# vislearn/esac

Measured on AMD Instinct MI355X. Metric: pose hypotheses/sec @640x480, 256 hyp, higher is better.
Workload: dtype f64 (P3P, LM refinement, exact decisions) + f32 (streaming soft-inlier score, ranking only); 1 GPU; BASELINE configs[1]: 1 expert(s), 256 hypotheses in total (256 per GPU), 60x80 grid (sub-sampling 8 of a 640x480 frame), all hypotheses on the one expert; tau=10 alpha=100 beta=0.5 maxReproj=100; box-room frames, 2 cm noise, 30% outliers; experts=1, hypotheses_total=256, frames_cycled=16, policy=range

## Files before the change

### esac_amd/api.py

```python
import ctypes as C
import os
import threading

import numpy as np
import torch

from . import build as _build

RES_SCORE, RES_HYP, RES_EXPERT, RES_RVEC, RES_TVEC, RES_POSE = 0, 1, 2, 3, 6, 9
RES_REF_STEPS, RES_INLIERS, RES_PROB, RES_ENTROPY, RES_CONTENDERS, RES_LM_ITERS, RES_DOUBLES = 25, 26, 27, 28, 29, 30, 32
BUF_HYPS, BUF_SAMPLE_XY, BUF_TRIES, BUF_SCORES, BUF_RESULT = 0, 1, 2, 3, 4
BUF_INLIER_MAP, BUF_INLIER_COUNTS, BUF_WINNER_ERRS, BUF_EXACT_FLAGS, BUF_CYCLES = 5, 6, 7, 8, 9
BUF_BWD_PROBS, BUF_BWD_LOSSES, BUF_BWD_REF_HYPS, BUF_BWD_SCORE_GRADS, BUF_BWD_SLOTS, BUF_BWD_SLOT_INFO, BUF_BWD_DLOSS = \
    10, 11, 12, 13, 14, 15, 16
BUF_BWD_PATH1, BUF_BWD_PATH2 = 17, 18
BUF_REFINE_INFO = 19
BUF_BWD_TEAM_INFO = 20
BUF_SPEC_INFO = 21
BUF_SPEC_FLAGS = 22
REFINE_TEAM_MAX, REFINE_TEAM_EIGHT, REFINE_TEAM_AUTO = 32, 8, -1
REFINE_TEAM_DEFAULT = REFINE_TEAM_AUTO
MAX_REF_STEPS = 100
BWD_MAX_SLOTS = 1000

ABI_SYMBOLS = [
    "esac_hip_abi_version", "esac_hip_last_error", "esac_hip_device_count", "esac_hip_create", "esac_hip_destroy",
    "esac_hip_forward", "esac_hip_sample", "esac_hip_score", "esac_hip_select", "esac_hip_refine",
    "esac_hip_score_exact", "esac_hip_read", "esac_hip_write_hyps", "esac_hip_phase_ms", "esac_hip_set_timing",
    "esac_hip_score_span_ms", "esac_hip_forward_batch", "esac_hip_backward", "esac_hip_set_debug", "esac_hip_check",
    "esac_hip_pick_record", "esac_hip_time_stages", "esac_hip_shard_balanced", "esac_hip_set_wait",
    "esac_hip_set_refine_team", "esac_hip_host_turn",
    "esac_hip_comm_unique_id", "esac_hip_comm_init", "esac_hip_comm_destroy", "esac_hip_allreduce_sum", "esac_hip_comm_info",
    "esac_hip_host_turn_mean", "esac_hip_backward_batch",
    "esac_hip_forward_batch_cams", "esac_hip_backward_batch_cams",
]
COMM_ID_BYTES = 128
ABI_VERSION = 6
FLAG_EXACT_SCORES, FLAG_SCORE_TILED, FLAG_SCORE_STREAM, FLAG_PACK_MAPS, FLAG_EXACT_SAMPLING, FLAG_SCORES_BY_INDEX = 1, 2, 4, 8, 16, 32
FLAG_AUTO_EXACT = 64
FLAG_REFINE_SOLO = 128
FLAG_STRICT_REFERENCE = 256
FLAG_STRICT_TRAINING = 512
WAIT_SPIN, WAIT_YIELD, WAIT_BLOCK = 0, 1, 2
DEBUG_ERROR_IMAGE, DEBUG_COOP_STALL, DEBUG_TEAM_SPREAD, DEBUG_NO_SPECULATION, DEBUG_SPEC_SECOND_BEST, DEBUG_SPEC_LOSE_CHAIN = 1, 2, 4, 8, 16, 32


class Params(C.Structure):
    _fields_ = [
        ("E", C.c_int32), ("H", C.c_int32), ("W", C.c_int32), ("N", C.c_int32),
        ("shift_x", C.c_int32), ("shift_y", C.c_int32),
        ("focal", C.c_float), ("ppx", C.c_float), ("ppy", C.c_float),
        ("inlier_thresh", C.c_float), ("inlier_alpha", C.c_float), ("inlier_beta", C.c_float),
        ("max_reproj", C.c_float), ("sub_sampling", C.c_int32),
        ("seed", C.c_uint64), ("call", C.c_uint64),
        ("max_tries", C.c_int32), ("max_ref_steps", C.c_int32), ("hyp_offset", C.c_int32),
        ("rescore_margin", C.c_float),
        ("d_hyp_index", C.c_void_p),
        ("flags", C.c_int32),
        ("expert_base", C.c_int32),
    ]


class FrameCam(C.Structure):
    _fields_ = [
        ("shift_x", C.c_int32), ("shift_y", C.c_int32),
        ("focal", C.c_float), ("ppx", C.c_float), ("ppy", C.c_float),
        ("reserved", C.c_int32 * 3),
    ]


CAM_DTYPE = np.dtype([("shift_x", np.int32), ("shift_y", np.int32), ("focal", np.float32), ("ppx", np.float32),
                      ("ppy", np.float32), ("reserved", np.int32, (3,))])


def make_cams(shift_x, shift_y, focal, ppx, ppy):
    B = len(shift_x)
    cams = np.zeros(B, CAM_DTYPE)
# ... 314 lines not shown

    def pick_record(self, records, world, zero=None):
        assert records.is_cuda and records.dtype == torch.float64 and records.is_contiguous() and records.numel() >= 32 * world
        assert zero is None or (zero.is_cuda and zero.dtype == torch.float64 and zero.is_contiguous())
        rc = self.lib.esac_hip_pick_record(self.ctx, records.data_ptr(), int(world), self._stream(), self._host_addr,
                                           zero.data_ptr() if zero is not None else None, int(zero.numel()) if zero is not None else 0)
        if rc != 0:
            _check(rc, self.lib)
        return self._host_np.copy()

    def shard_balanced(self, hyp_assign, world, rank, E, expert_base=0, index_out=None, assign_out=None, info_out=None):
        assert hyp_assign.is_cuda and hyp_assign.dtype == torch.int64 and hyp_assign.is_contiguous()
        N = int(hyp_assign.shape[0])
        n_local = N // world + (1 if rank < N % world else 0)
        dev = self.device
        if index_out is None:
            index_out = torch.empty(max(n_local, 1), dtype=torch.int32, device=dev)
        if assign_out is None:
            assign_out = torch.empty(max(n_local, 1), dtype=torch.int64, device=dev)
        if info_out is None:
            info_out = torch.empty(4, dtype=torch.int32, device=dev)
        self._call(self.lib.esac_hip_shard_balanced, hyp_assign.data_ptr(), N, int(E), int(world), int(rank), int(expert_base),
                   self._stream(), index_out.data_ptr(), assign_out.data_ptr(), info_out.data_ptr())
        self._keep_shard = (hyp_assign, index_out, assign_out, info_out)
        return index_out[:n_local], assign_out[:n_local], info_out

    def set_wait(self, mode):
        _check(self.lib.esac_hip_set_wait(self.ctx, int(mode)), self.lib)

    def check(self):
        _check(self.lib.esac_hip_check(self.ctx), self.lib)

    def set_debug(self, keep_error_image=False, coop_stall=False, team_spread=False, no_speculation=False, spec_second_best=False,
                  spec_lose_chain=False):
        _check(self.lib.esac_hip_set_debug(self.ctx, (DEBUG_ERROR_IMAGE if keep_error_image else 0) | (DEBUG_COOP_STALL if coop_stall else 0) |
                                           (DEBUG_TEAM_SPREAD if team_spread else 0) | (DEBUG_NO_SPECULATION if no_speculation else 0) |
                                           (DEBUG_SPEC_SECOND_BEST if spec_second_best else 0) | (DEBUG_SPEC_LOSE_CHAIN if spec_lose_chain else 0)), self.lib)

    def spec_info(self):
        v = self.read(BUF_SPEC_INFO)
        return {"calls": int(v[0]), "failures": int(v[1]), "last_speculative": bool(v[2]), "last_failed": bool(v[3])}

    def set_refine_team(self, members=REFINE_TEAM_DEFAULT):
        _check(self.lib.esac_hip_set_refine_team(self.ctx, int(members)), self.lib)

    def bwd_team_info(self):
        v = self.read(BUF_BWD_TEAM_INFO)
        return {"teams": bool(v[0]), "team_calls": int(v[1]), "team_fallbacks": int(v[2]), "slots": int(v[3])}

    def refine_info(self):
        v = self.read(BUF_REFINE_INFO)
        return {"mode": ("one_workgroup", "cooperating", "team")[int(v[0])] if 0 <= int(v[0]) <= 2 else int(v[0]),
                "workgroups": int(v[1]),
                "xcd_census": [(int(v[2]) >> (8 * x)) & 255 for x in range(4)] + [(int(v[7]) >> (8 * x)) & 255 for x in range(4)],
                "same_xcd": bool(v[3]),
                "exchanges": int(v[4]), "timed_out": bool(v[5]), "team_fallbacks": int(v[6]) & 0x3fffffff,
                "team_latched_off": bool(int(v[6]) & 0x40000000)}

    def comm_unique_id(self):
        buf = (C.c_ubyte * COMM_ID_BYTES)()
        _check(self.lib.esac_hip_comm_unique_id(buf, COMM_ID_BYTES), self.lib)
        return bytes(buf)

    def comm_init(self, nranks, rank, unique_id):
        assert len(unique_id) == COMM_ID_BYTES
        buf = (C.c_ubyte * COMM_ID_BYTES).from_buffer_copy(unique_id)
        _check(self.lib.esac_hip_comm_init(self.ctx, int(nranks), int(rank), buf, COMM_ID_BYTES), self.lib)
        self._comm = (int(nranks), int(rank))

    def comm_destroy(self):
# ... 308 lines not shown
```

### esac_amd/csrc/esac_capi.hip

```cpp
#include <hip/hip_runtime.h>
#include <dlfcn.h>
#include <sched.h>
#include <time.h>
#include <stdarg.h>
#include <stddef.h>
#include <stdio.h>
#include <stdlib.h>
#include <string.h>

#include "../../include/esac_hip.h"
#include "esac_kernels.hpp"
#include "pose_math.hpp"

using namespace esac;

extern "C" {
typedef struct ncclComm* ncclComm_t;
typedef struct { char internal[128]; } ncclUniqueId;
typedef int ncclResult_t;
}

static_assert(ESAC_RES_SCORE == ESAC_RES_SCORE_K && ESAC_RES_HYP == ESAC_RES_HYP_K && ESAC_RES_EXPERT == ESAC_RES_EXPERT_K &&
                  ESAC_RES_RVEC == ESAC_RES_RVEC_K && ESAC_RES_POSE == ESAC_RES_POSE_K &&
                  ESAC_RES_REF_STEPS == ESAC_RES_REF_STEPS_K && ESAC_RES_INLIERS == ESAC_RES_INLIERS_K &&
// ... 71 lines not shown
    int last_nsel = 0;
    bool slot_teams = true;
    long long slot_team_calls = 0, slot_team_fallbacks = 0;
    bool last_bwd_teams = false;
    BwdArgs bws{};
    int bP = 0, bcap = 0;
    long long bN = 0, bslots = 0, brows = 0;
    int bB = 0;
    bool b_lists = false;
    int bcap_batch = 0;
    long long bwd_budget = 2048LL << 20;
    int last_bwd_frames = 1;
    int last_bwd_batch_cap = 0;
    double* h_gt = nullptr;
    double* d_gt = nullptr;
    FrameCam* h_cams = nullptr;
    FrameCam* d_cams = nullptr;
    hipEvent_t cams_ev = nullptr;
    bool cams_queued = false;
    float4* sc4 = nullptr;
    long long sc4_cells = 0;
    int tN = 0, tChunks = 0;
    long long tPart = 0;
    bool rt32_stale = false;
    double host_ns[8] = {0, 0, 0, 0, 0, 0, 0, 0};
    double host_sum[8] = {0, 0, 0, 0, 0, 0, 0, 0};
    double host_last_return = 0;
    long long host_n = 0;
    hipStream_t side = nullptr;
    hipStream_t side2 = nullptr;
    bool spec_off = false, spec_env_off = false;
    bool spec_second_best = false;
    bool spec_lose_chain = false;
    long long spec_calls = 0;
    double last_spec_epoch = 0;
    ncclComm_t comm = nullptr;
    int comm_ranks = 0, comm_rank = 0;
};

static inline double now_ns() {
    timespec ts;
    clock_gettime(CLOCK_MONOTONIC, &ts);
    return (double)ts.tv_sec * 1e9 + (double)ts.tv_nsec;
}

extern "C" int esac_hip_abi_version(void) { return ESAC_HIP_ABI_VERSION; }
extern "C" const char* esac_hip_last_error(void) { return g_err; }
extern "C" int esac_hip_device_count(void) {
    int n = 0;
    if (hipGetDeviceCount(&n) != hipSuccess) return 0;
    return n;
}

constexpr int ESAC_SLOT_TEAMS_MAX = 32;
constexpr int ESAC_TEAM_STRIKES = 2;
constexpr long long ESAC_TEAM_REARM_CALLS = 1000;

static_assert(sizeof(ncclUniqueId) == ESAC_COMM_ID_BYTES, "unique id size");
constexpr ncclResult_t ncclSuccess = 0;
constexpr int NCCL_SUM = 0, NCCL_DOUBLE = 8;
struct Rccl {
    ncclResult_t (*get_unique_id)(ncclUniqueId*) = nullptr;
    ncclResult_t (*comm_init_rank)(ncclComm_t*, int, ncclUniqueId, int) = nullptr;
    ncclResult_t (*comm_destroy)(ncclComm_t) = nullptr;
    ncclResult_t (*all_reduce)(const void*, void*, size_t, int, int, ncclComm_t, hipStream_t) = nullptr;
    const char* (*error_string)(ncclResult_t) = nullptr;
// ... 554 lines not shown
        KArgs as = a;
        as.spec_mode = 1;
        as.result_user = nullptr;
        as.result_pin = nullptr;
        launch_score(as, s);
        if ((rc = check_launch("k_score_fast (settled)"))) return rc;
        c->host_ns[2] = now_ns() - t_entry;
        if (tm) HIP_OK(hipEventRecord(c->ev[2], s));
        if (tm) HIP_OK(hipEventRecord(c->ev[3], s));
        KArgs ar = as;
        ar.spec_mode = 2;
        ar.spec_debug = c->spec_second_best ? 1 : 0;
        c->refine_tag = launch_refine(ar, s);
        c->refine_was_team = refine_team_members(ar) > 0;
        if ((rc = check_launch("k_refine (speculative)"))) return rc;
        launch_spec_wait(a, 3, c->side2);
        launch_select_rescore(as, c->side2);
        if ((rc = check_launch("k_select_rescore (settled)"))) return rc;
        launch_spec_wait(a, 3, c->side);
        launch_sample_stragglers_on(chain, chain_waves, c->side);
        if (!c->spec_lose_chain) launch_score_stragglers(a, c->side);
        if ((rc = check_launch("straggler chain"))) return rc;
        launch_spec_join(a, c->side2);
        if ((rc = check_launch("k_spec_join"))) return rc;
        {
            KArgs ag = a;
            ag.spec_gate = 1;
            const unsigned long long tag2 = launch_refine(ag, s);
            (void)tag2;
            if ((rc = check_launch("k_refine (gated)"))) return rc;
        }
        c->host_ns[3] = now_ns() - t_entry;
    } else {
        launch_sample(a, s);
        if ((rc = check_launch("k_sample"))) return rc;
        c->host_ns[1] = now_ns() - t_entry;
        if (tm) HIP_OK(hipEventRecord(c->ev[1], s));
        if (exact) launch_rescore_all(a, s);
        else       launch_score(a, s);
        if ((rc = check_launch(exact ? "k_rescore(all)" : "k_score_fast"))) return rc;
        c->host_ns[2] = now_ns() - t_entry;
        if (tm) HIP_OK(hipEventRecord(c->ev[2], s));
        a.fold_select = !c->fold_select ? 0 : refine_folds_select(a) ? 1 : refine_folds_exact_stats(a) ? 2 : 0;
        if (exact) {
            if (a.fold_select != 2) launch_stats_exact(a, s);
        } else if (!a.fold_select) {
            launch_select_rescore(a, s);
        }
        if ((rc = check_launch(exact ? "k_stats_exact" : "k_select_rescore"))) return rc;
        if (tm) HIP_OK(hipEventRecord(c->ev[3], s));
        c->refine_tag = launch_refine(a, s);
        c->refine_was_team = refine_team_members(a) > 0;
        if ((rc = check_launch("k_refine"))) return rc;
        c->host_ns[3] = now_ns() - t_entry;
    }
    if (tm) {
        HIP_OK(hipEventRecord(c->ev[4], s));
        HIP_OK(hipEventRecord(c->ev[5], s));
        HIP_OK(hipEventRecord(c->ev[6], s));
        c->ev_valid = true;
    }
    if (h_result_out) {
        if ((rc = wait_record(c, s, B, c->epoch, "esac_hip_forward: the refinement kernel"))) return rc;
        if (spec_ok && c->h_pin[33] == 5.0) {
            c->spec_off = c->spec_env_off = true;
            HIP_OK(hipStreamSynchronize(c->side));
            if (c->side2) HIP_OK(hipStreamSynchronize(c->side2));
            HIP_OK(hipStreamSynchronize(s));
            return forward_impl(c, d_sc, sc_frame_stride, d_assign, p, B, stream, d_scores_out, d_result_out, h_result_out);
        }
        c->host_ns[4] = now_ns() - t_entry;
        bool team_failed = false;
// ... 49 lines not shown
    for (int k = 0; k < 6; k++) out_ns[k] = c->host_sum[k] / n;
    out_ns[6] = c->host_n > 1 ? c->host_sum[6] / (double)(c->host_n - 1) : 0.0;
    out_ns[7] = (double)c->host_n;
    if (reset) {
        for (double& v : c->host_sum) v = 0;
        c->host_n = 0;
        c->host_last_return = 0;
    }
    return 0;
}

extern "C" int esac_hip_host_turn(esac_hip_ctx* c, double out_ns[8]) {
    if (!c || !out_ns) return fail(-1, "esac_hip_host_turn: null argument");
    for (int k = 0; k < 8; k++) out_ns[k] = c->host_ns[k];
    return 0;
}

extern "C" int esac_hip_time_stages(esac_hip_ctx* c, const float* d_sc, const int64_t* d_assign, const esac_hip_params* p,
                                    void* stream, int reps, float out_ms[4]) {
    if (!c || !out_ms || reps < 1) return fail(-1, "esac_hip_time_stages: bad argument");
    DeviceGuard guard(c->device);
    KArgs a;
    int rc = make_args(c, d_sc, d_assign, p, &a);
    if (rc) return rc;
    a.tstamps = nullptr;
    forward_team(c, a);
    hipStream_t s = (hipStream_t)stream;
    c->rt32_stale = false;
    mark_sampling(c, a);
    if ((a.flags & ESAC_FLAG_AUTO_EXACT) && a.E == 1 && (long long)a.N * a.H * a.W <= ESAC_AUTO_EXACT_MAX_WORK)
        a.flags |= ESAC_FLAG_EXACT_SCORES | ESAC_FLAG_EXACT_SAMPLING;
    const bool exact = (a.flags & ESAC_FLAG_EXACT_SCORES) != 0;
    a.fold_select = !c->fold_select ? 0 : refine_folds_select(a) ? 1 : refine_folds_exact_stats(a) ? 2 : 0;
    auto stage = [&](int k) {
        switch (k) {
            case 0: launch_sample(a, s); break;
            case 1: if (exact) launch_rescore_all(a, s); else launch_score(a, s); break;
            case 2: if (exact) { if (a.fold_select != 2) launch_stats_exact(a, s); } else if (!a.fold_select) launch_select_rescore(a, s); break;
            default: c->refine_tag = launch_refine(a, s); break;
        }
    };
    for (int k = 0; k < 4; k++) stage(k);
    if ((rc = check_launch("forward chain"))) return rc;
    hipEvent_t ev[8];
    for (auto& e : ev) HIP_OK(hipEventCreate(&e));
    for (int k = 0; k < 4; k++) {
        stage(k);
        HIP_OK(hipEventRecord(ev[2 * k], s));
        for (int r = 0; r < reps; r++) stage(k);
        HIP_OK(hipEventRecord(ev[2 * k + 1], s));
    }
    if ((rc = check_launch("stage timing"))) return rc;
    HIP_OK(hipEventSynchronize(ev[7]));
    for (int k = 0; k < 4; k++) {
        HIP_OK(hipEventElapsedTime(&out_ms[k], ev[2 * k], ev[2 * k + 1]));
        out_ms[k] /= (float)reps;
    }
    for (auto& e : ev) (void)hipEventDestroy(e);
    return 0;
}

extern "C" int esac_hip_pick_record(esac_hip_ctx* c, const double* d_records, int world, void* stream, double* h_record_out, double* d_zero,
                                    int n_zero) {
    if (!c || !d_records || !h_record_out || world < 1 || n_zero < 0 || (n_zero > 0 && !d_zero))
        return fail(-1, "esac_hip_pick_record: bad argument");
    DeviceGuard guard(c->device);
    hipStream_t s = (hipStream_t)stream;
    c->epoch += 1.0;
    const double want = c->epoch;
// ... 562 lines not shown

extern "C" int esac_hip_write_hyps(esac_hip_ctx* c, const double* h_hyps, int N) {
    if (!c || !h_hyps || N <= 0) return fail(-1, "esac_hip_write_hyps: bad argument");
    DeviceGuard guard(c->device);
    int rc = ensure_ws(c, N, c->capP > 0 ? c->capP : 1);
    if (rc) return rc;
    HIP_OK(hipDeviceSynchronize());
    HIP_OK(hipMemcpy(c->ws.hyps, h_hyps, (size_t)N * 6 * sizeof(double), hipMemcpyHostToDevice));
    c->rt32_stale = true;
    c->lastN = N;
    return 0;
}

extern "C" int esac_hip_set_refine_team(esac_hip_ctx* c, int members) {
    if (!c) return fail(-1, "null context");
    if (members < ESAC_REFINE_TEAM_AUTO || members > ESAC_REFINE_TEAM_MAX)
        return fail(-4, "esac_hip_set_refine_team: %d members (0..%d, or ESAC_REFINE_TEAM_AUTO)", members, ESAC_REFINE_TEAM_MAX);
    c->team_auto = members == ESAC_REFINE_TEAM_AUTO && !c->team_auto_env_off;
    c->team = members == ESAC_REFINE_TEAM_AUTO ? ESAC_REFINE_TEAM_DEFAULT : members < 2 ? 0 : members;
    c->team_latched_off = false;
    c->team_strikes = 0;
    c->slot_teams = true;
    return 0;
}

extern "C" int esac_hip_set_debug(esac_hip_ctx* c, int flags) {
    if (!c) return fail(-1, "null context");
    c->keep_errs = (flags & ESAC_DEBUG_ERROR_IMAGE) != 0;
    c->coop_stall = (flags & ESAC_DEBUG_COOP_STALL) != 0;
    c->team_spread = (flags & ESAC_DEBUG_TEAM_SPREAD) != 0;
    c->spec_off = c->spec_env_off || (flags & ESAC_DEBUG_NO_SPECULATION) != 0;
    c->spec_second_best = (flags & ESAC_DEBUG_SPEC_SECOND_BEST) != 0;
    c->spec_lose_chain = (flags & ESAC_DEBUG_SPEC_LOSE_CHAIN) != 0;
    return 0;
}

extern "C" int esac_hip_set_timing(esac_hip_ctx* c, int enabled) {
    if (!c) return fail(-1, "null context");
    c->timing = enabled != 0;
    c->timing_period = enabled > 1 ? enabled : 1;
    c->timing_calls = 0;
    c->ev_valid = false;
    if (c->ws.span_acc) {
        DeviceGuard guard(c->device);
        HIP_OK(hipDeviceSynchronize());
        HIP_OK(hipMemset(c->ws.span_acc, 0, 2 * sizeof(long long)));
    }
    return 0;
}

extern "C" int esac_hip_phase_ms(esac_hip_ctx* c, float out[6]) {
    if (!c || !out) return fail(-1, "esac_hip_phase_ms: null argument");
    if (!c->timing || !c->ev_valid) return fail(-8, "esac_hip_phase_ms: timing is off or no forward has run");
    DeviceGuard guard(c->device);
    HIP_OK(hipEventSynchronize(c->ev[4]));
    for (int i = 0; i < 4; i++) HIP_OK(hipEventElapsedTime(&out[i], c->ev[i], c->ev[i + 1]));
    HIP_OK(hipEventElapsedTime(&out[4], c->ev[0], c->ev[4]));
    HIP_OK(hipEventSynchronize(c->ev[6]));
    HIP_OK(hipEventElapsedTime(&out[5], c->ev[5], c->ev[6]));
    return 0;
}

extern "C" int esac_hip_score_span_ms(esac_hip_ctx* c, float* mean_ms, int* launches) {
    if (!c || !mean_ms) return fail(-1, "esac_hip_score_span_ms: null argument");
    if (!c->ws.span_acc) return fail(-8, "esac_hip_score_span_ms: no forward has run");
    DeviceGuard guard(c->device);
// ... 8 lines not shown
```

### esac_amd/csrc/esac_kernels.hip

```cpp
#include <hip/hip_runtime.h>
#include <stdint.h>
#include <stdlib.h>

#include "pose_math.hpp"
#include "p3p_screen.hpp"
#include "rng.hpp"
#include "esac_kernels.hpp"
#include "device_common.hpp"

namespace esac {

__device__ __forceinline__ bool accept_sample(const double Rp[9], const double Tp[3], const float (&Pf)[4][3], const double (&mu)[4],
                                              const double (&mv)[4], const Cam& cam, double tau, double rvec[3], double T[3],
                                              double R[9]) {
    rodrigues_mat2vec(Rp, rvec);
    rodrigues_vec2mat<false>(rvec, R, nullptr);
    T[0] = Tp[0]; T[1] = Tp[1]; T[2] = Tp[2];
    bool accepted = true;
#pragma unroll
    for (int j = 0; j < 4; j++) {
        const double Xd = Pf[j][0], Yd = Pf[j][1], Zd = Pf[j][2];
        double x = R[0] * Xd + R[1] * Yd + R[2] * Zd + T[0];
        double y = R[3] * Xd + R[4] * Yd + R[5] * Zd + T[1];
        double z = R[6] * Xd + R[7] * Yd + R[8] * Zd + T[2];
// ... 1014 lines not shown
        double R[9];
#pragma unroll
        for (int k = 0; k < 9; k++) R[k] = a.hyps_R[(size_t)h * 9 + k];
        double acc[1] = {0};
        for (int i = threadIdx.x; i < P; i += B) {
            const int row = i / a.W, col = i - row * a.W;
            float err = project_exact_err(R, t, cam, mx[i], mx[P + i], mx[2 * P + i], cell_px(a, col), cell_py(a, row));
            if (STRICT) err = a.max_reproj < err ? a.max_reproj : err;
            else        err = err < a.max_reproj ? err : a.max_reproj;
            acc[0] += soft_inlier_exact(err, a.tau, a.beta);
        }
        block_sum<1, B>(acc, s_part, s_tot);
        if (threadIdx.x == 0) {
            const float scale = a.alpha / a.W / a.H;
            double s = acc[0];
            s *= scale;
            a.scores[h] = s;
            if (a.scores_user) a.scores_user[user_slot(a, h)] = s;
            a.exact_flag[h] = 1;
        }
        __syncthreads();
    }
}

template <int B>
__global__ __launch_bounds__(B) void k_rescore(KArgs a) {
    rescore_body<B, false>(a);
}
template <int B>
__global__ __launch_bounds__(B) void k_rescore_strict(KArgs a) {
    rescore_body<B, true>(a);
}

template <int B>
__global__ __launch_bounds__(B) void k_stats_exact(KArgs a) {
    __shared__ double s_part[2 * (B / 64)];
    __shared__ double s_tot[2];
    __shared__ double s_max[B / 64];
    frame_view(a);
    double m = -INFINITY;
    for (int i = threadIdx.x; i < a.N; i += B) m = fmax(m, a.scores[i]);
#pragma unroll
    for (int o = 32; o > 0; o >>= 1) m = fmax(m, __shfl_xor(m, o));
    if ((threadIdx.x & 63) == 0) s_max[threadIdx.x >> 6] = m;
    __syncthreads();
    m = s_max[0];
#pragma unroll
    for (int k = 1; k < B / 64; k++) m = fmax(m, s_max[k]);
    double acc[2] = {0, 0};
    for (int i = threadIdx.x; i < a.N; i += B) {
        const double d = a.scores[i] - m;
        const double ex = exp(d);
        acc[0] += ex;
        acc[1] += ex * d;
    }
    block_sum<2, B>(acc, s_part, s_tot);
    if (threadIdx.x == 0) {
        a.n_contenders[0] = a.N;
        a.stats[0] = m;
        a.stats[1] = acc[0];
        a.stats[2] = log2(acc[0]) - acc[1] / (acc[0] * 0.6931471805599453);
    }
}

template <int B>
__global__ __launch_bounds__(B) void k_stats_strict(KArgs a) {
// ... 217 lines not shown
    if (total <= (handover ? ESAC_LATENCY_MAX : 1024)) {
        if (handover) b.handover = ESAC_HANDOVER;
        if (total <= 256)                    hipLaunchKernelGGL((strict ? k_sample_strict<256, 2> : k_sample<256, 2>), dim3(a.N, a.frames), dim3(256), 0, s, b);
        else if (total <= 512 || !handover)  hipLaunchKernelGGL((strict ? k_sample_strict<128, 4> : k_sample<128, 4>), dim3(a.N, a.frames), dim3(128), 0, s, b);
        else                                 hipLaunchKernelGGL((k_sample<64, 2>), dim3(a.N, a.frames), dim3(64), 0, s, b);
    } else if (total <= 4096 && !handover) {
        hipLaunchKernelGGL((strict ? k_sample_strict<128, 1> : k_sample<128, 1>), dim3(a.N, a.frames), dim3(128), 0, s, b);
    } else {
        if (total <= ESAC_FIRST_WIDE_MAX) {
            hipLaunchKernelGGL((strict ? k_sample_first_strict<32> : k_sample_first<32>), dim3((a.N + 1) / 2, a.frames), dim3(64), 0, s, b);
            b.first_try += 32;
        } else if (a.E > 1 && !exact) {
        } else {
            for (int pass = 0; pass < FIRST_PHASE_TRIES / 16 && b.first_try < a.max_tries; pass++) {
                hipLaunchKernelGGL((strict ? k_sample_first_strict<16> : k_sample_first<16>), dim3((a.N + 3) / 4, a.frames), dim3(64), 0, s, b);
                b.first_try += 16;
            }
        }
        if (b.first_try < a.max_tries) {
            if (exact) {
                hipLaunchKernelGGL((strict ? k_sample_strict<64, 1> : k_sample<64, 1>), dim3(a.N, a.frames), dim3(64), 0, s, b);
            } else {
                hipLaunchKernelGGL(k_pending_list, dim3((a.N + 1023) / 1024, a.frames), dim3(1024), 0, s, b);
                launch_sample_stragglers(b, waves, s);
            }
        }
        return;
    }
    if (handover) {
        b.first_try = b.handover;
        launch_sample_stragglers(b, waves, s);
    }
}
constexpr int ESAC_SPLIT_LATENCY_MAX = 1024, ESAC_SPLIT_HANDOVER = 32;
bool sample_can_split(const KArgs& a) {
    return a.frames == 1 && a.E > 1 && a.max_tries > 1024 && !(a.flags & (ESAC_FLAG_EXACT_SAMPLING_K | ESAC_FLAG_STRICT_REFERENCE_K)) && a.N <= ESAC_FIRST_WIDE_MAX &&
           a.first_try == 0;
}
int launch_sample_split(const KArgs& a, hipStream_t s, KArgs* chain, int* chain_waves) {
    const long long total = a.N;
    if (a.sc4) hipLaunchKernelGGL(k_pack_cells, dim3(2048), dim3(256), 0, s, a);
    KArgs b = a;
    b.handover = 0x7fffffff;
    const long long w8 = (long long)8 * total;
    *chain_waves = (int)(w8 < ESAC_CHAIN_WAVES ? ESAC_CHAIN_WAVES : (w8 > 131072 ? 131072 : w8));
    if (total <= ESAC_SPLIT_LATENCY_MAX) {
        b.handover = ESAC_SPLIT_HANDOVER;
        if (total <= 256)      hipLaunchKernelGGL((k_sample<256, 2>), dim3(a.N, 1), dim3(256), 0, s, b);
        else if (total <= 512) hipLaunchKernelGGL((k_sample<128, 4>), dim3(a.N, 1), dim3(128), 0, s, b);
        else                   hipLaunchKernelGGL((k_sample<64, 2>), dim3(a.N, 1), dim3(64), 0, s, b);
        b.first_try = b.handover;
    } else {
        hipLaunchKernelGGL(k_sample_first<32>, dim3((a.N + 1) / 2, 1), dim3(64), 0, s, b);
        b.first_try += 32;
        hipLaunchKernelGGL(k_pending_list, dim3((a.N + 1023) / 1024, 1), dim3(1024), 0, s, b);
    }
    *chain = b;
    return 0;
}
void launch_sample_stragglers_on(const KArgs& chain, int waves, hipStream_t side) { launch_sample_stragglers(chain, waves, side); }
void launch_score_stragglers(const KArgs& a, hipStream_t side) {
    KArgs b = a;
    b.tstamps = nullptr;
    b.spec_mode = 0;
    const int grid = a.N < 1024 ? a.N : 1024;
    if ((long long)a.N <= 2048) hipLaunchKernelGGL(k_score_stragglers<512>, dim3(grid), dim3(512), 0, side, b);
// ... 33 lines not shown
```

### esac_amd/csrc/esac_kernels.hpp

```cpp
#pragma once
#include <hip/hip_runtime.h>
#include <stdint.h>

namespace esac {

constexpr int ESAC_RES_SCORE_K = 0, ESAC_RES_HYP_K = 1, ESAC_RES_EXPERT_K = 2, ESAC_RES_RVEC_K = 3,
              ESAC_RES_POSE_K = 9, ESAC_RES_REF_STEPS_K = 25, ESAC_RES_INLIERS_K = 26, ESAC_RES_PROB_K = 27,
              ESAC_RES_ENTROPY_K = 28, ESAC_RES_CONTENDERS_K = 29, ESAC_RES_LM_ITERS_K = 30;
constexpr int ESAC_MAX_REF_STEPS_K = 100;
constexpr int ESAC_BWD_SLOTS_K = 1000;
constexpr int ESAC_REFINE_LDS_CAP = 8192;
constexpr int ESAC_REFINE_THREADS = 256;
constexpr int ESAC_ERR_UNROLL = 8;
constexpr int ESAC_REFINE_COOP_MAX = 256;
constexpr int ESAC_REFINE_TEAM_DEFAULT_K = 8;
constexpr int ESAC_REFINE_TEAM_MAX_K = 32;
constexpr int ESAC_REFINE_TEAM_MIN_CELLS = 1024;
constexpr int ESAC_TEAM_BATCH_MAX = 32;
constexpr int ESAC_TEAM_GRANULES = 2 * ESAC_REFINE_TEAM_MAX_K * 32;
constexpr long ESAC_TEAM_SPIN_LIMIT = 100000, ESAC_TEAM_SPIN_LIMIT_SLOTS = 800000;
constexpr int ESAC_PIN_DOUBLES = 36;
__host__ __device__ inline unsigned long long pin_mix(unsigned long long bits, int k) {
    const unsigned long long h = (bits + (unsigned long long)(k + 1) * 0x9E3779B97F4A7C15ull) * 0xD6E8FEB86659FD93ull;
    const int r = k & 63;
// ... 61 lines not shown
    int pad_[3];
};
static_assert(sizeof(FrameCam) == 32, "one aligned 32-byte record per frame");

struct KArgs {
    const float* sc;
    const int64_t* assign;
    int E, H, W, N;
    int shift_x, shift_y, sub;
    float focal, ppx, ppy;
    float tau, alpha, beta, max_reproj;
    uint64_t seed, call;
    int max_tries, max_ref_steps, hyp_offset;
    int first_try;
    int handover;
    float margin;
    int flags;
    int expert_base;
    const int32_t* hyp_index;
    double* hyps;
    double* hyps_R;
    float* rt32;
    int* sample_xy;
    int* tries;
    const float4* sc4;
    int* samp_resume;
    int* samp_round;
    unsigned long long* best_try;
    double* samp_cand;
    int* samp_entries;
    int* samp_count;
    int* samp_pending;
    int samp_cap;
    float* fast_scores;
    double* scores;
    uint8_t* exact_flag;
    int* n_contenders;
    double* sel_partials;
    int* sel_arrived;
    double* stats;
    float* errs;
    uint8_t* inlier_map;
    void* corr_list;
    int* inlier_counts;
    double* result;
    long long* cycles;
    long long* tstamps;
    long long* span_acc;
    unsigned long long* status;
    double* coop_partials;
    unsigned long long* coop_counter;
    int coop_slice;
    int coop_max;
    int coop_extra;
    unsigned long long coop_tag;
    int team;
    int team_auto;
    int team_stride;
    int solo;
    int* refine_info;
    int fold_select;
    int spec_mode;
    uint8_t* spec_flag;
    double* spec_state;
    int* spec_cnt;
    int spec_gate;
// ... 13 lines not shown
    int frames;
    long long sc_frame_stride;
    const FrameCam* cams;
    BwdArgs bwd;
};

void launch_sample(const KArgs& a, hipStream_t s);
bool sample_can_split(const KArgs& a);
int launch_sample_split(const KArgs& a, hipStream_t s, KArgs* chain, int* chain_waves);
void launch_sample_stragglers_on(const KArgs& chain, int waves, hipStream_t side);
void launch_score_stragglers(const KArgs& a, hipStream_t side);
void launch_spec_join(const KArgs& a, hipStream_t s);
void launch_spec_wait(const KArgs& a, int which, hipStream_t s);
void launch_hyps_to_rt32(const KArgs& a, hipStream_t s);
void launch_score_fast(const KArgs& a, hipStream_t s);
void launch_score(const KArgs& a, hipStream_t s);
void launch_score_tiled(const KArgs& a, hipStream_t s);
void launch_bucket_order(const KArgs& a, hipStream_t s);
int tiled_sub_tiles(int P);
void launch_select_rescore(const KArgs& a, hipStream_t s);
void launch_rescore_all(const KArgs& a, hipStream_t s, bool per_frame_shape = false);
void launch_stats_exact(const KArgs& a, hipStream_t s);
void launch_pick_record(const double* records, int world, double* pin, double epoch, double* zero, int n_zero, hipStream_t s);
void launch_shard_balanced(const int64_t* assign, int N, int E, int world, int rank, int expert_base, int32_t* index_out,
                           int64_t* assign_out, int32_t* info_out, hipStream_t s);
int refine_coop_capacity();
int refine_coop_slice(const KArgs& a);
int refine_team_members(const KArgs& a);
unsigned long long launch_refine(const KArgs& a, hipStream_t s);
unsigned long long launch_refine_team(const KArgs& a, hipStream_t s);
unsigned long long next_refine_tag();
bool refine_folds_select(const KArgs& a);
bool refine_folds_exact_stats(const KArgs& a);
void launch_refine_slots(const KArgs& a, hipStream_t s);
bool refine_slots_can_team(const KArgs& a);
unsigned long long launch_refine_slots_team(KArgs& a, hipStream_t s);
void launch_bwd_select(const KArgs& a, hipStream_t s);
void launch_bwd_loss(const KArgs& a, hipStream_t s);
void launch_bwd_paths(const KArgs& a, hipStream_t s);
void launch_bwd_accumulate(const KArgs& a, hipStream_t s);
__host__ __device__ inline int bwd_rows(int N) { return N < ESAC_BWD_SLOTS_K ? N : ESAC_BWD_SLOTS_K; }

}
```

### esac_amd/csrc/sample_kernels.inc.hpp

```cpp

template <int TRIES>
__global__ __launch_bounds__(64) ESAC_SAMPLE_FIRST_ATTR void ESAC_K_SAMPLE_FIRST(KArgs a) {
    constexpr int HPW = 64 / TRIES;
    frame_view(a);
    const int lane = threadIdx.x, grp = lane / TRIES, t = a.first_try + (lane & (TRIES - 1));
    const int h = blockIdx.x * HPW + grp;
    const int hc = h < a.N ? h : a.N - 1;
    const bool mine_pending = h < a.N && (a.first_try == 0 || a.tries[hc] == SAMPLE_PENDING);
    if (!__any(mine_pending)) return;
    const bool active = mine_pending && t < a.max_tries;
    if (a.first_try == 0 && h < a.N && (lane & (TRIES - 1)) == 0) flag_bad_assignment(a, h);
    const int e = expert_of(a, hc);
    const int P = a.H * a.W;
    const float* __restrict__ map = a.sc + (size_t)e * 3 * P;
    const Philox rng(a.seed, a.call);
    const Cam cam = make_cam(a);
    int cx[4] = {0, 0, 0, 0}, cy[4] = {0, 0, 0, 0};
    double rvec[3] = {0, 0, 0}, T[3] = {0, 0, 0};
    double R[9] = {1, 0, 0, 0, 1, 0, 0, 0, 1};
    bool accepted = false;
    if (active) {
        V3 Pt[4];
        float Pf[4][3];
        double mu[4], mv[4], Rp[9], Tp[3];
        gather_sample(a, map, P, rng, (uint32_t)global_hyp(a, hc), (uint32_t)t, cx, cy, Pt, Pf, mu, mv);
        double reproj2 = 0;
        if (p3p_4pt<ESAC_SAMPLE_ALIGN>(Pt, mu, mv, cam, Rp, Tp, &reproj2) && (t == a.max_tries - 1 || !cannot_pass(reproj2, (double)a.tau)))
            accepted = accept_sample(Rp, Tp, Pf, mu, mv, cam, (double)a.tau, rvec, T, R);
    }
    const unsigned long long m = __ballot(accepted);
    const unsigned mine = (unsigned)(m >> (TRIES * grp)) & (TRIES == 32 ? 0xffffffffu : 0xffffu);
    if (mine_pending) {
        if (mine) {
            const int first = __ffs((int)mine) - 1;
            if ((lane & (TRIES - 1)) == first) store_hypothesis(a, h, map, rvec, T, R, cx, cy, a.first_try + first);
        } else if (a.max_tries <= a.first_try + TRIES) {
            if (t == a.max_tries - 1) store_hypothesis(a, h, map, rvec, T, R, cx, cy, -1);
        } else if ((lane & (TRIES - 1)) == 0) {
            a.tries[h] = SAMPLE_PENDING;
        }
    }
}

template <int SAMPLE_B, int LPT>
__global__ __launch_bounds__(SAMPLE_B) void ESAC_K_SAMPLE(KArgs a) {
    static_assert(LPT == 1 || LPT == 2 || LPT == 4, "lanes per try");
    constexpr int CPLN = 4 / LPT;
    __shared__ int s_first[2][SAMPLE_B / 64];
    __shared__ double s_pose[CPLN > 1 ? SAMPLE_B * 12 : 1];
    frame_view(a);
    const int h = blockIdx.x;
    const int lane = threadIdx.x & 63, wave = threadIdx.x >> 6;
    const int e = expert_of(a, h);
    const int P = a.H * a.W;
    const float* __restrict__ map = a.sc + (size_t)e * 3 * P;
    const Philox rng(a.seed, a.call);
    const Cam cam = make_cam(a);
    const uint32_t gh = (uint32_t)global_hyp(a, h);
    const double tau = (double)a.tau;
    if (a.first_try > 0 && a.tries[h] != SAMPLE_PENDING) return;
    if (a.first_try == 0 && threadIdx.x == 0) flag_bad_assignment(a, h);
    if (a.handover != 0x7fffffff && threadIdx.x == 0 && expert_stats_on(a)) atomicAdd(expert_stats(a, e), 1);

    int parity = 0;
    for (int base = a.first_try, TRIES = 0; base < a.max_tries; base += TRIES, parity ^= 1) {
        const bool quad = LPT > 1 && base < SAMPLE_B;
        TRIES = quad ? SAMPLE_B / LPT : SAMPLE_B;
        const int t = base + (quad ? (int)threadIdx.x / LPT : (int)threadIdx.x);
        const int sub = threadIdx.x & (LPT - 1);
        bool holder = !quad;
        const bool active = t < a.max_tries;
        int cx[4] = {0, 0, 0, 0}, cy[4] = {0, 0, 0, 0};
        double rvec[3] = {0, 0, 0}, T[3] = {0, 0, 0};
        double R[9] = {1, 0, 0, 0, 1, 0, 0, 0, 1};
        bool accepted = false;
// ... 45 lines not shown
#pragma unroll
                    for (int q = 0; q < 9; q++) Rp[q] = s_pose[q * SAMPLE_B + threadIdx.x];
#pragma unroll
                    for (int q = 0; q < 3; q++) Tp[q] = s_pose[(9 + q) * SAMPLE_B + threadIdx.x];
                }
                holder = solved || (!have && sub == 0);
                reproj2 = min_reproj;
            } else {
                solved = p3p_4pt<ESAC_SAMPLE_ALIGN>(Pt, mu, mv, cam, Rp, Tp, &reproj2);
            }
            if (solved && (t == a.max_tries - 1 || !cannot_pass(reproj2, tau)))
                accepted = accept_sample(Rp, Tp, Pf, mu, mv, cam, tau, rvec, T, R);
        }
        const unsigned long long m = __ballot(accepted);
        if (lane == 0) {
            const int first_lane = __ffsll((long long)m) - 1;
            s_first[parity][wave] = m ? base + (quad ? wave * (64 / LPT) + first_lane / LPT : wave * 64 + first_lane) : 0x7fffffff;
        }
        __syncthreads();
        int first = s_first[parity][0];
#pragma unroll
        for (int w = 1; w < SAMPLE_B / 64; w++) first = min(first, s_first[parity][w]);
        const bool last_round = base + TRIES >= a.max_tries;
        int writer = -1, tries_val = -1;
        if (first != 0x7fffffff) {
            writer = first;
            tries_val = first;
        } else if (last_round) {
            writer = a.max_tries - 1;
        }
        if (writer >= 0) {
            if (t == writer && holder) store_hypothesis(a, h, map, rvec, T, R, cx, cy, tries_val);
            if (a.spec_flag && threadIdx.x == 0) a.spec_flag[h] = 0;
            return;
        }
        if (base + TRIES >= a.handover) {
            if (threadIdx.x < 64) mark_pending(a, h, e, threadIdx.x == 0);
            return;
        }
    }
}
```

### include/esac_hip.h

```cpp
#ifndef ESAC_HIP_H
#define ESAC_HIP_H

#include <stddef.h>
#include <stdint.h>

#ifdef __cplusplus
extern "C" {
#endif

#define ESAC_HIP_ABI_VERSION 6

#define ESAC_MAX_SAMPLING_TRIES 1000000
#define ESAC_MAX_REF_STEPS 100
#define ESAC_MAX_BATCH 1024

typedef struct esac_hip_params {
    int32_t E, H, W;
    int32_t N;
    int32_t shift_x, shift_y;
    float focal, ppx, ppy;
    float inlier_thresh;
    float inlier_alpha;
    float inlier_beta;
    float max_reproj;
// ... 122 lines not shown
                                 const float* h_gt_poses, const esac_hip_frame_cam* h_cams, float w_loss_rot,
                                 float w_loss_trans, float loss_cut, const esac_hip_params* p, void* stream, double* h_out);

int esac_hip_sample(esac_hip_ctx* ctx, const float* d_scene_coords, const int64_t* d_hyp_assign,
                    const esac_hip_params* p, void* stream);
int esac_hip_score(esac_hip_ctx* ctx, const float* d_scene_coords, const int64_t* d_hyp_assign,
                   const esac_hip_params* p, void* stream);
int esac_hip_select(esac_hip_ctx* ctx, const float* d_scene_coords, const int64_t* d_hyp_assign,
                    const esac_hip_params* p, void* stream);
int esac_hip_refine(esac_hip_ctx* ctx, const float* d_scene_coords, const int64_t* d_hyp_assign,
                    const esac_hip_params* p, void* stream);

int esac_hip_score_exact(esac_hip_ctx* ctx, const float* d_scene_coords, const int64_t* d_hyp_assign,
                         const esac_hip_params* p, void* stream);

int esac_hip_check(esac_hip_ctx* ctx);

int esac_hip_read(esac_hip_ctx* ctx, int which, void* h_dst, size_t bytes);
int esac_hip_write_hyps(esac_hip_ctx* ctx, const double* h_hyps, int N);

int esac_hip_phase_ms(esac_hip_ctx* ctx, float out[6]);
int esac_hip_score_span_ms(esac_hip_ctx* ctx, float* mean_ms, int* launches);
int esac_hip_time_stages(esac_hip_ctx* ctx, const float* d_scene_coords, const int64_t* d_hyp_assign,
                         const esac_hip_params* p, void* stream, int reps, float out_ms[4]);
int esac_hip_host_turn(esac_hip_ctx* ctx, double out_ns[8]);
int esac_hip_host_turn_mean(esac_hip_ctx* ctx, double out_ns[8], int reset);
int esac_hip_set_timing(esac_hip_ctx* ctx, int enabled);
#define ESAC_DEBUG_ERROR_IMAGE 1
#define ESAC_DEBUG_COOP_STALL 2
#define ESAC_DEBUG_TEAM_SPREAD 4
#define ESAC_DEBUG_NO_SPECULATION 8
#define ESAC_DEBUG_SPEC_SECOND_BEST 16
#define ESAC_DEBUG_SPEC_LOSE_CHAIN 32
int esac_hip_set_debug(esac_hip_ctx* ctx, int flags);

#define ESAC_REFINE_TEAM_MAX 32
#define ESAC_REFINE_TEAM_DEFAULT 8
#define ESAC_REFINE_TEAM_AUTO (-1)
int esac_hip_set_refine_team(esac_hip_ctx* ctx, int members);

#define ESAC_WAIT_SPIN 0
#define ESAC_WAIT_YIELD 1
#define ESAC_WAIT_BLOCK 2
int esac_hip_set_wait(esac_hip_ctx* ctx, int mode);

#ifdef __cplusplus
}
#endif
#endif
```

Baseline: 2.643 million hypotheses/s.

## Fuse exact scoring into the sampling kernel for single-frame exact runs

Adds a k_sample_score kernel variant. Once a workgroup settles on its hypothesis, it passes R and t through shared memory and immediately computes that hypothesis's exact soft-inlier score over all cells, so the separate rescore-all launch is skipped. This removes one kernel launch and the re-read of the hypotheses between stages. In exchange, scoring is tied to the sampling grid of one workgroup per hypothesis, which can leave the GPU underused when sampling is uneven. A debug flag turns the fusion off.

```diff
diff --git a/esac_amd/api.py b/esac_amd/api.py
--- a/esac_amd/api.py
+++ b/esac_amd/api.py
@@ -43,6 +43,7 @@
 FLAG_STRICT_TRAINING = 512
 WAIT_SPIN, WAIT_YIELD, WAIT_BLOCK = 0, 1, 2
 DEBUG_ERROR_IMAGE, DEBUG_COOP_STALL, DEBUG_TEAM_SPREAD, DEBUG_NO_SPECULATION, DEBUG_SPEC_SECOND_BEST, DEBUG_SPEC_LOSE_CHAIN = 1, 2, 4, 8, 16, 32
+DEBUG_NO_FUSED_SCORE = 64
 
 
 class Params(C.Structure):
@@ -423,10 +424,11 @@
         _check(self.lib.esac_hip_check(self.ctx), self.lib)
 
     def set_debug(self, keep_error_image=False, coop_stall=False, team_spread=False, no_speculation=False, spec_second_best=False,
-                  spec_lose_chain=False):
+                  spec_lose_chain=False, no_fused_score=False):
         _check(self.lib.esac_hip_set_debug(self.ctx, (DEBUG_ERROR_IMAGE if keep_error_image else 0) | (DEBUG_COOP_STALL if coop_stall else 0) |
                                            (DEBUG_TEAM_SPREAD if team_spread else 0) | (DEBUG_NO_SPECULATION if no_speculation else 0) |
-                                           (DEBUG_SPEC_SECOND_BEST if spec_second_best else 0) | (DEBUG_SPEC_LOSE_CHAIN if spec_lose_chain else 0)), self.lib)
+                                           (DEBUG_SPEC_SECOND_BEST if spec_second_best else 0) | (DEBUG_SPEC_LOSE_CHAIN if spec_lose_chain else 0) |
+                                           (DEBUG_NO_FUSED_SCORE if no_fused_score else 0)), self.lib)
 
     def spec_info(self):
         v = self.read(BUF_SPEC_INFO)
diff --git a/esac_amd/csrc/esac_capi.hip b/esac_amd/csrc/esac_capi.hip
--- a/esac_amd/csrc/esac_capi.hip
+++ b/esac_amd/csrc/esac_capi.hip
@@ -127,6 +127,7 @@
     bool spec_off = false, spec_env_off = false;
     bool spec_second_best = false;
     bool spec_lose_chain = false;
+    bool no_fused_score = false;
     long long spec_calls = 0;
     double last_spec_epoch = 0;
     ncclComm_t comm = nullptr;
@@ -747,12 +748,15 @@
         }
         c->host_ns[3] = now_ns() - t_entry;
     } else {
-        launch_sample(a, s);
+        const bool fused = exact && B == 1 && !c->no_fused_score && sample_fuses_score(a);
+        if (fused) launch_sample_score(a, s);
+        else       launch_sample(a, s);
         if ((rc = check_launch("k_sample"))) return rc;
         c->host_ns[1] = now_ns() - t_entry;
         if (tm) HIP_OK(hipEventRecord(c->ev[1], s));
-        if (exact) launch_rescore_all(a, s);
-        else       launch_score(a, s);
+        if (fused)      {}
+        else if (exact) launch_rescore_all(a, s);
+        else            launch_score(a, s);
         if ((rc = check_launch(exact ? "k_rescore(all)" : "k_score_fast"))) return rc;
         c->host_ns[2] = now_ns() - t_entry;
         if (tm) HIP_OK(hipEventRecord(c->ev[2], s));
@@ -868,9 +872,10 @@
         a.flags |= ESAC_FLAG_EXACT_SCORES | ESAC_FLAG_EXACT_SAMPLING;
     const bool exact = (a.flags & ESAC_FLAG_EXACT_SCORES) != 0;
     a.fold_select = !c->fold_select ? 0 : refine_folds_select(a) ? 1 : refine_folds_exact_stats(a) ? 2 : 0;
+    const bool fused = exact && !c->no_fused_score && sample_fuses_score(a);
     auto stage = [&](int k) {
         switch (k) {
-            case 0: launch_sample(a, s); break;
+            case 0: if (fused) launch_sample_score(a, s, false); else launch_sample(a, s); break;
             case 1: if (exact) launch_rescore_all(a, s); else launch_score(a, s); break;
             case 2: if (exact) { if (a.fold_select != 2) launch_stats_exact(a, s); } else if (!a.fold_select) launch_select_rescore(a, s); break;
             default: c->refine_tag = launch_refine(a, s); break;
@@ -1499,6 +1504,7 @@
     c->spec_off = c->spec_env_off || (flags & ESAC_DEBUG_NO_SPECULATION) != 0;
     c->spec_second_best = (flags & ESAC_DEBUG_SPEC_SECOND_BEST) != 0;
     c->spec_lose_chain = (flags & ESAC_DEBUG_SPEC_LOSE_CHAIN) != 0;
+    c->no_fused_score = (flags & ESAC_DEBUG_NO_FUSED_SCORE) != 0;
     return 0;
 }
 
diff --git a/esac_amd/csrc/esac_kernels.hip b/esac_amd/csrc/esac_kernels.hip
--- a/esac_amd/csrc/esac_kernels.hip
+++ b/esac_amd/csrc/esac_kernels.hip
@@ -1070,6 +1070,102 @@
     rescore_body<B, true>(a);
 }
 
+__device__ __forceinline__ double* score_hand() {
+    __shared__ double s_hand[12];
+    return s_hand;
+}
+template <int SAMPLE_B>
+__device__ __forceinline__ void score_sampled(const KArgs& a, int h) {
+    constexpr int VB = 1024, ACC = VB / SAMPLE_B;
+    static_assert(ACC * SAMPLE_B == VB && SAMPLE_B % 64 == 0, "whole virtual wavefronts per real wavefront");
+    __shared__ double s_part[VB / 64];
+    const double* s_hand = score_hand();
+    long long t_start = 0;
+    if (a.tstamps && threadIdx.x == 0) t_start = wall_clock64();
+    __syncthreads();
+    const int P = a.H * a.W;
+    const Cam cam = make_cam(a);
+    const float* __restrict__ mx = a.sc + (size_t)expert_of(a, h) * 3 * P;
+    double R[9];
+#pragma unroll
+    for (int k = 0; k < 9; k++) R[k] = s_hand[k];
+    const double t[3] = {s_hand[9], s_hand[10], s_hand[11]};
+    const int lane = threadIdx.x & 63, wave = threadIdx.x >> 6;
+    double acc[ACC];
+#pragma unroll
+    for (int j = 0; j < ACC; j++) acc[j] = 0;
+    const int step_row = VB / a.W, step_col = VB - step_row * a.W;
+    int row[ACC], col[ACC];
+#pragma unroll
+    for (int j = 0; j < ACC; j++) {
+        const int c = 64 * (ACC * wave + j) + lane;
+        row[j] = c / a.W;
+        col[j] = c - row[j] * a.W;
+    }
+    for (int base = 64 * ACC * wave + lane; base < P; base += VB) {
+        double v[ACC];
+#pragma unroll
+        for (int j = 0; j < ACC; j++) {
+            const int c = base + 64 * j;
+            const int i = c < P ? c : P - 1;
+            float err = project_exact_err(R, t, cam, mx[i], mx[P + i], mx[2 * P + i], cell_px(a, col[j]), cell_py(a, row[j]));
+            err = err < a.max_reproj ? err : a.max_reproj;
+            v[j] = soft_inlier_exact(err, a.tau, a.beta);
+            col[j] += step_col;
+            row[j] += step_row;
+            if (col[j] >= a.W) {
+                col[j] -= a.W;
+                row[j] += 1;
+            }
+        }
+#pragma unroll
+        for (int j = 0; j < ACC; j++) {
+            const double sum = acc[j] + v[j];
+            acc[j] = base + 64 * j < P ? sum : acc[j];
+        }
+    }
+#pragma unroll
+    for (int j = 0; j < ACC; j++) {
+        const double w = wave_sum(acc[j]);
+        if (lane == 0) s_part[ACC * wave + j] = w;
+    }
+    __syncthreads();
+    if (threadIdx.x == 0) {
+        double s = 0;
+#pragma unroll
+        for (int w = 0; w < VB / 64; w++) s += s_part[w];
+        const float scale = a.alpha / a.W / a.H;
+        s *= scale;
+        a.scores[h] = s;
+        if (a.scores_user) a.scores_user[user_slot(a, h)] = s;
+        a.exact_flag[h] = 1;
+        if (a.tstamps) {
+            a.tstamps[2 * h] = t_start;
+            a.tstamps[2 * h + 1] = wall_clock64();
+        }
+    }
+}
+#define ESAC_K_SAMPLE k_sample_score
+#define ESAC_SAMPLE_ALIGN AlignTriad
+#define ESAC_SAMPLE_NO_FIRST
+#define ESAC_SAMPLE_SETTLED(mine, R, T)                        \
+    {                                                          \
+        if (mine) {                                            \
+            double* s_hand = score_hand();                     \
+            for (int q = 0; q < 9; q++) s_hand[q] = (R)[q];    \
+            for (int q = 0; q < 3; q++) s_hand[9 + q] = (T)[q]; \
+        }                                                      \
+        break;                                                 \
+    }
+#define ESAC_SAMPLE_EPILOGUE \
+    if (a.score_in_sample && a.first_try < a.max_tries) score_sampled<SAMPLE_B>(a, h);
+#include "sample_kernels.inc.hpp"
+#undef ESAC_K_SAMPLE
+#undef ESAC_SAMPLE_ALIGN
+#undef ESAC_SAMPLE_NO_FIRST
+#undef ESAC_SAMPLE_SETTLED
+#undef ESAC_SAMPLE_EPILOGUE
+
 template <int B>
 __global__ __launch_bounds__(B) void k_stats_exact(KArgs a) {
     __shared__ double s_part[2 * (B / 64)];
@@ -1353,6 +1449,19 @@
         launch_sample_stragglers(b, waves, s);
     }
 }
+bool sample_fuses_score(const KArgs& a) {
+    const bool strict = (a.flags & ESAC_FLAG_STRICT_REFERENCE_K) != 0;
+    const bool handover = a.E > 1 && a.max_tries > 1024 && !(a.flags & ESAC_FLAG_EXACT_SAMPLING_K);
+    return (a.flags & ESAC_FLAG_EXACT_SCORES_K) != 0 && !strict && a.frames == 1 && a.first_try == 0 && a.N <= 256 && !handover &&
+           (long long)a.N * a.H * a.W <= (1LL << 21);
+}
+void launch_sample_score(const KArgs& a, hipStream_t s, bool score) {
+    if (a.sc4) hipLaunchKernelGGL(k_pack_cells, dim3(2048), dim3(256), 0, s, a);
+    KArgs b = a;
+    b.handover = 0x7fffffff;
+    b.score_in_sample = score ? 1 : 0;
+    hipLaunchKernelGGL((k_sample_score<256, 2>), dim3(a.N, 1), dim3(256), 0, s, b);
+}
 constexpr int ESAC_SPLIT_LATENCY_MAX = 1024, ESAC_SPLIT_HANDOVER = 32;
 bool sample_can_split(const KArgs& a) {
     return a.frames == 1 && a.E > 1 && a.max_tries > 1024 && !(a.flags & (ESAC_FLAG_EXACT_SAMPLING_K | ESAC_FLAG_STRICT_REFERENCE_K)) && a.N <= ESAC_FIRST_WIDE_MAX &&
diff --git a/esac_amd/csrc/esac_kernels.hpp b/esac_amd/csrc/esac_kernels.hpp
--- a/esac_amd/csrc/esac_kernels.hpp
+++ b/esac_amd/csrc/esac_kernels.hpp
@@ -117,6 +117,7 @@
     int* samp_count;
     int* samp_pending;
     int samp_cap;
+    int score_in_sample;
     float* fast_scores;
     double* scores;
     uint8_t* exact_flag;
@@ -196,6 +197,8 @@
 unsigned long long next_refine_tag();
 bool refine_folds_select(const KArgs& a);
 bool refine_folds_exact_stats(const KArgs& a);
+bool sample_fuses_score(const KArgs& a);
+void launch_sample_score(const KArgs& a, hipStream_t s, bool score = true);
 void launch_refine_slots(const KArgs& a, hipStream_t s);
 bool refine_slots_can_team(const KArgs& a);
 unsigned long long launch_refine_slots_team(KArgs& a, hipStream_t s);
diff --git a/esac_amd/csrc/sample_kernels.inc.hpp b/esac_amd/csrc/sample_kernels.inc.hpp
--- a/esac_amd/csrc/sample_kernels.inc.hpp
+++ b/esac_amd/csrc/sample_kernels.inc.hpp
@@ -1,4 +1,10 @@
+#ifndef ESAC_SAMPLE_SETTLED
+#define ESAC_SAMPLE_SETTLED(mine, R, T) return;
+#define ESAC_SAMPLE_EPILOGUE
+#define ESAC_SAMPLE_PLAIN_
+#endif
 
+#ifndef ESAC_SAMPLE_NO_FIRST
 template <int TRIES>
 __global__ __launch_bounds__(64) ESAC_SAMPLE_FIRST_ATTR void ESAC_K_SAMPLE_FIRST(KArgs a) {
     constexpr int HPW = 64 / TRIES;
@@ -41,6 +47,8 @@
         }
     }
 }
+
+#endif
 
 template <int SAMPLE_B, int LPT>
 __global__ __launch_bounds__(SAMPLE_B) void ESAC_K_SAMPLE(KArgs a) {
@@ -152,11 +160,17 @@
         if (writer >= 0) {
             if (t == writer && holder) store_hypothesis(a, h, map, rvec, T, R, cx, cy, tries_val);
             if (a.spec_flag && threadIdx.x == 0) a.spec_flag[h] = 0;
-            return;
+            ESAC_SAMPLE_SETTLED(t == writer && holder, R, T)
         }
         if (base + TRIES >= a.handover) {
             if (threadIdx.x < 64) mark_pending(a, h, e, threadIdx.x == 0);
             return;
         }
     }
+    ESAC_SAMPLE_EPILOGUE
 }
+#ifdef ESAC_SAMPLE_PLAIN_
+#undef ESAC_SAMPLE_SETTLED
+#undef ESAC_SAMPLE_EPILOGUE
+#undef ESAC_SAMPLE_PLAIN_
+#endif
diff --git a/include/esac_hip.h b/include/esac_hip.h
--- a/include/esac_hip.h
+++ b/include/esac_hip.h
@@ -178,6 +178,7 @@
 #define ESAC_DEBUG_NO_SPECULATION 8
 #define ESAC_DEBUG_SPEC_SECOND_BEST 16
 #define ESAC_DEBUG_SPEC_LOSE_CHAIN 32
+#define ESAC_DEBUG_NO_FUSED_SCORE 64
 int esac_hip_set_debug(esac_hip_ctx* ctx, int flags);
 
 #define ESAC_REFINE_TEAM_MAX 32
```

Result: slower. 2.390 million hypotheses/s (-9.6%).
